# oliver-batchelor/multical

Measured on AMD Instinct MI355X. Metric: residual+Jacobian evals/sec, higher is better.
Workload: dtype f64; 1 GPU; BASELINE configs[2]: 8 cameras x 500 frames x 2 boards (charuco_16x22 + aprilgrid_9x9), rolling-shutter motion, intrinsics+extrinsics; the whole rig on 1 GPU(s); n_params=6140, n_slots=2592000, n_observations=763957, parallelism=single GPU, device=gfx950:sramecc+:xnack-:AMD Radeon Graphics:cus=256:mfma=1

## Files before the change

### multical_amd/_lib.py

```python
import ctypes as C
import os

import numpy as np

HERE = os.path.dirname(os.path.abspath(__file__))
LIB_PATH = os.environ.get("MCBA_LIB_PATH") or os.path.join(HERE, "_build", "libmcba.so")

MCBA_VERSION = 3
MOTION_STATIC, MOTION_ROLLING, MOTION_HAND_EYE = 0, 1, 2
CAMERA_PINHOLE, CAMERA_FISHEYE = 0, 1
LOSSES = dict(linear=0, soft_l1=1, huber=2, cauchy=3, arctan=4)
TR_SOLVERS = dict(exact=0, lsmr=1)
OPT_BITS = dict(camera_poses=1, board_poses=2, motion=4, cameras=8, boards=16)
PARAM_ORDER = ["camera_poses", "board_poses", "motion", "cameras", "boards"]

c_double_p = C.POINTER(C.c_double)
c_uint8_p = C.POINTER(C.c_uint8)
c_int32_p = C.POINTER(C.c_int32)


class Problem(C.Structure):
  _fields_ = [
    ("version", C.c_int32), ("n_cameras", C.c_int32), ("n_frames", C.c_int32), ("n_boards", C.c_int32),
    ("n_points", C.c_int32),
# ... 235 lines not shown
                                              c_double_p, C.POINTER(C.c_int64), c_double_p]),
  ("mcba_debug_observation_covariance_ms", C.c_int32, [H, c_double_p]),
  ("mcba_debug_set_observation_covariance_route", C.c_int32, [H, C.c_int32]),
  ("mcba_residual_gram", C.c_int32, [H, c_double_p, c_int32_p, C.c_int32, C.c_int32, C.c_int32, C.c_int32, c_double_p,
                                     C.POINTER(C.c_int64), C.POINTER(C.c_int64), C.c_int32, C.c_int32, c_int32_p]),
  ("mcba_debug_residual_gram_ms", C.c_int32, [c_double_p, C.POINTER(C.c_int64)]),
  ("mcba_warp_points", C.c_int32, [C.POINTER(FieldSet), C.c_int64, c_int32_p, C.c_int32, c_double_p, c_double_p, c_uint8_p]),
  ("mcba_undistort_maps_corrected", C.c_int32, [C.POINTER(CameraSet), C.POINTER(FieldSet), c_double_p, c_double_p, C.c_int32, C.c_int32,
                                                C.POINTER(C.c_float)]),
  ("mcba_undistort_images_corrected", C.c_int32, [C.POINTER(CameraSet), C.POINTER(FieldSet), c_double_p, c_double_p, C.c_void_p,
                                                  C.c_int32, C.c_int32, C.c_int32, C.c_int32, C.c_int32, c_int32_p, C.c_int32, C.c_int32,
                                                  C.c_double, C.c_void_p]),
  ("mcba_debug_warp_ms", C.c_int32, [c_double_p, C.POINTER(C.c_int64)]),
  ("mcba_solve", C.c_int32, [H, c_double_p, C.POINTER(Options), C.POINTER(Result)]),
  ("mcba_time_linearize", C.c_int32, [H, c_double_p, C.POINTER(Options), C.c_int32, c_double_p]),
  ("mcba_time_residuals", C.c_int32, [H, c_double_p, C.c_int32, c_double_p]),
  ("mcba_time_lsmr_iteration", C.c_int32, [H, c_double_p, C.c_int32, c_double_p]),
  ("mcba_rccl_unique_id", C.c_int32, [C.POINTER(C.c_uint8)]),
  ("mcba_rccl_init", C.c_int32, [H, C.POINTER(C.c_uint8), C.c_int32, C.c_int32]),
  ("mcba_rccl_shutdown", C.c_int32, [H]),
  ("mcba_rccl_version", C.c_int32, [C.POINTER(C.c_int32)]),
  ("mcba_set_mfma", C.c_int32, [H, C.c_int32]),
  ("mcba_debug_set_lin_grid", C.c_int32, [H, C.c_int32]),
  ("mcba_debug_set_frame_groups", C.c_int32, [H, C.c_int32]),
  ("mcba_debug_pipe_probe", C.c_int32, [C.c_int32, C.POINTER(C.c_double)]),
  ("mcba_debug_dot3", C.c_int32, [C.POINTER(C.c_double), C.POINTER(C.c_double), C.c_int64, C.POINTER(C.c_double), C.POINTER(C.c_double)]),
  ("mcba_debug_dispatch_probe", C.c_int32, [C.c_int32, C.c_int32, C.c_int32, C.c_int32, C.POINTER(C.c_longlong)]),
  ("mcba_debug_xcd_probe", C.c_int32, [C.c_int32, C.POINTER(C.c_longlong)]),
  ("mcba_debug_gn_step", C.c_int32, [H, C.c_double, c_double_p, c_double_p, c_double_p]),
  ("mcba_debug_mfma_probe", C.c_int32, [c_double_p, c_double_p]),
  ("mcba_debug_chol", C.c_int32, [H, C.c_int32, c_double_p, c_double_p, C.c_double, C.c_int32, c_double_p]),
  ("mcba_debug_linearize_profile", C.c_int32, [H, c_double_p, C.POINTER(C.c_longlong)]),
  ("mcba_debug_lsmr_products", C.c_int32, [H, c_double_p, c_double_p, c_double_p, c_double_p, c_double_p]),
  ("mcba_debug_lsmr_fused_products", C.c_int32, [H, c_double_p, c_double_p, c_double_p, c_double_p]),
  ("mcba_debug_lsmr_info", C.c_int32, [H, C.POINTER(C.c_int64)]),
  ("mcba_debug_set_lsmr_fused", C.c_int32, [H, C.c_int32]),
  ("mcba_debug_set_switch", C.c_int32, [C.c_char_p, C.c_char_p]),
  ("mcba_debug_lsmr_solve", C.c_int32, [H, c_double_p, C.POINTER(Options), C.c_double, c_double_p, C.c_int32, c_double_p, c_double_p, c_double_p]),
  ("mcba_debug_lsmr_trace", C.c_int32, [H, C.c_int32, c_double_p, C.POINTER(C.c_int32)]),
  ("mcba_debug_set_lsmr_trace", C.c_int32, [H, C.c_int32]),
  ("mcba_debug_set_lsmr_grid", C.c_int32, [H, C.c_int32]),
  ("mcba_debug_set_allreduce_trace", C.c_int32, [H, C.c_int32]),
  ("mcba_debug_set_lsmr_masks_form", C.c_int32, [H, C.c_int32]),
]

_lib = None
# ... 69 lines not shown
```

### multical_amd/backend.py

```python
import ctypes as C
import time
from types import SimpleNamespace

import numpy as np

from . import _lib
from ._lib import (Problem, Options, Result, RoundReport, LOSSES, OPT_BITS, PARAM_ORDER, MOTION_STATIC, MOTION_ROLLING,
                   MOTION_HAND_EYE, CAMERA_PINHOLE, CAMERA_FISHEYE, check, f64 as _f64)


def _ptr(a, ctype):
  return a.ctypes.data_as(C.POINTER(ctype))


def _mask_u8(a):
  a = np.asarray(a)
  if a.dtype == np.bool_ and a.flags.c_contiguous:
    return a.view(np.uint8)
  if a.dtype == np.uint8 and a.flags.c_contiguous:
    return a
  return np.ascontiguousarray(a.astype(np.uint8))


def _class_name(obj):
# ... 141 lines not shown

  def __enter__(self):
    return self

  def __exit__(self, *a):
    self.close()

  @property
  def n_residuals(self):
    n = C.c_int64()
    check(self.lib.mcba_num_residuals(self.h, C.byref(n)))
    return n.value

  def device_info(self):
    buf = C.create_string_buffer(256)
    check(self.lib.mcba_device_info(self.h, buf, 256))
    return buf.value.decode()

  def set_mfma(self, on):
    check(self.lib.mcba_set_mfma(self.h, 1 if on else 0))

  def set_lin_grid(self, grid):
    check(self.lib.mcba_debug_set_lin_grid(self.h, int(grid)))

  def set_frame_groups(self, nw):
    check(self.lib.mcba_debug_set_frame_groups(self.h, int(nw)))

  def set_inliers(self, mask):
    self._jac_pattern = None
    if mask is None:
      check(self.lib.mcba_set_inliers(self.h, None))
    else:
      m = _mask_u8(mask)
      assert m.shape == tuple(self.shape), f"inlier mask shape {m.shape} != {self.shape}"
      check(self.lib.mcba_set_inliers(self.h, _ptr(m, C.c_uint8)))

  def _x(self, x):
    x = _f64(x)
    assert x.shape == (self.n_params,), f"inconsistent parameter sizes, got {x.size}, expected {self.n_params}"
    return x

  def residuals(self, x):
    x = self._x(x)
    r = np.empty(self.n_residuals)
    check(self.lib.mcba_residuals(self.h, _ptr(x, C.c_double), _ptr(r, C.c_double)))
    return r
# ... 430 lines not shown
```

### multical_amd/csrc/mcba_api.hip

```cpp
#include <dlfcn.h>
#include <cmath>
#include <limits>

#include "../../include/mcba.h"
#include "mcba_debug.h"
#include "mcba_camops.h"
#include "mcba_dispatch.h"
#include "mcba_lower.h"
#include "mcba_solver_kernels.h"
#include "mcba_cov_kernels.h"
#include "mcba_obscov_kernels.h"
#include "mcba_residual_field_kernels.h"
#include "mcba_host.h"

using namespace mcba;
using namespace mcba::host;

namespace mcba {
namespace host {
thread_local std::string g_error;
__thread hipStream_t g_fill_stream = nullptr;
__thread bool g_park_on_release = false;
ResourceCache& resource_cache() {
  static ResourceCache* c = new ResourceCache();
  return *c;
}
}
}

static std::map<std::string, std::string>& dbg_switch_table() {
  static std::map<std::string, std::string> t;
  return t;
}
static std::mutex g_dbg_switch_mutex;
const char* mcba::host::dbg_switch(const char* name) {
  {
// ... 69 lines not shown
  DevBuf<double> comm;
  DevBuf<double> ls_u, ls_ua, ls_ub, ls_part, ls_v, ls_vraw, ls_h, ls_hbar, ls_x, ls_nrm, ls_partial, ls_out, ls_bpart, ls_comm, ls_xpart, ls_vpart, ls_part2;
  DevBuf<double2> cp_obs, cp_bxy;
  DevBuf<double> cp_bz, cp_tr;
  DevBuf<double> dot_part;
  DevBuf<int4> cp_desc;
  bool compact_dirty = true;
  DevBuf<double> ls_cache;
  int lsmr_fused_setting = -1;
  bool lsmr_masks_form = false;
  int lsmr_fused = 2;
  ScalLayout sl;
  DevBuf<double> chol_linv;
  DevBuf<double> cov_d, cov_zero, cov_x, cov_p, cov_sg, cov_sout, cov_ff, cov_fs;
  DevBuf<int32_t> cov_bad;
  DevBuf<uint8_t> oc_flag;
  DevBuf<double> oc_cov, oc_student, oc_part, oc_out, oc_g;
  double oc_pass_ms = 0.0;
  bool oc_sigma_route = false;
  DevBuf<int32_t> rf_size, rf_cov;
  DevBuf<double> rf_part, rf_gram;
  DevBuf<long long> rf_cpart, rf_count;
  int lin_grid = 0;

  int64_t n_inliers = 0;
  int64_t n_evalid = 0;

  DevBuf<double2> obs;
  DevBuf<uint8_t> inlier, evalid, fix_aspect;
  DevBuf<uint8_t> valid_fm, raw_mask, cam_valid, frame_valid, board_valid;
  DevBuf<int32_t> view_first;
  DevBuf<long long> totals;
  long long* h_totals = nullptr;
  DevBuf<int32_t> obs_index, view_count, active_views, av_counts, work_counter, board_off, full2act;
  DevBuf<double> xfull, bwg, img_h, board_points, pose, cam, view, tmat;
  DevBuf<uint16_t> tri;
  DevBuf<int4> ftab;
  int nftab = 0;
  DevBuf<long long> dbg;
  DevBuf<double> err_fm, sel_f64;
  std::vector<double> err_x;
  bool err_valid = false;
  DevBuf<unsigned int> sel_hist;
  DevBuf<unsigned long long> sel_state;
  bool obs_index_dirty = false;
  bool view_first_dirty = false;
// ... 114 lines not shown
  const Dims& d = h->d;
  h->obs_index_dirty = true; h->compact_dirty = true;
  if (d.views() > 0) {
    if (mask_ref != nullptr) {
      if (h->raw_mask.n < (size_t)d.slots()) h->raw_mask.alloc((size_t)d.slots(), false);
      upload_shard_slabs(h, h->raw_mask.p, mask_ref, 1);
      hipLaunchKernelGGL(k_lower_view, dim3(d.views()), dim3(64), 0, h->stream, d, (const double2*)nullptr, (const float2*)nullptr,
                         (const uint8_t*)h->raw_mask.p, (const uint8_t*)h->raw_mask.p, h->cam_valid.p, h->frame_valid.p,
                         h->board_valid.p, h->board_off.p, (double2*)nullptr, (uint8_t*)nullptr, (uint8_t*)nullptr,
                         h->inlier.p, h->view_count.p, (int32_t*)nullptr);
    } else {
      hipLaunchKernelGGL(k_inliers_from_valid, dim3(d.views()), dim3(64), 0, h->stream, d, h->valid_fm.p, h->inlier.p,
                         h->view_count.p);
    }
  }
  refresh_active_views(h);
  scan_views(h);
  h->out_r.alloc((size_t)std::max<int64_t>(2 * h->n_inliers, 1), false);
}

void set_loss(mcba_handle_s* h, const mcba_options* opt) {
  h->d.loss = opt ? opt->loss : MCBA_LOSS_LINEAR;
  h->d.f_scale = opt ? opt->f_scale : 1.0;
  REQUIRE(h->d.loss >= 0 && h->d.loss <= 4, "unknown loss");
  REQUIRE(h->d.loss == 0 || h->d.f_scale > 0, "f_scale must be positive");
}

void upload_x(mcba_handle_s* h, const double* x, double* dst) {
  if (h->ext2int.empty()) {
    memcpy(h->h_x, x, (size_t)h->d.n * sizeof(double));
  } else {
    memset(h->h_x, 0, (size_t)h->d.n * sizeof(double));
    for (int i = 0; i < h->n_ext; ++i) h->h_x[h->ext2int[i]] = x[i];
  }
  HIP_OK(hipMemcpyAsync(dst, h->h_x, (size_t)h->d.n * sizeof(double), hipMemcpyHostToDevice, h->stream));
}

void eval_pose_tables(mcba_handle_s* h, const double* dx) {
  const Dims& d = h->d;
  const int items = d.n_pose + d.C + d.B * d.P;
  hipLaunchKernelGGL(k_prep, dim3((items + 127) / 128), dim3(128), 0, h->stream, d, h->t, dx);
}

void eval_tables(mcba_handle_s* h, const double* dx) {
  const Dims& d = h->d;
  eval_pose_tables(h, dx);
// ... 33 lines not shown
}
void destroy_rccl_comm(void* comm) {
  if (comm && rccl_api().ok) (void)rccl_api().CommDestroy(comm);
}
int32_t rccl_allreduce_native(void* ctx, void* device_buf, size_t count, int32_t op, void* stream) {
  mcba_handle_s* h = static_cast<mcba_handle_s*>(ctx);
  const int rc = rccl_api().AllReduce(device_buf, device_buf, count,  8, op == 0 ?  0 :  2,
                                      h->rccl_comm, (hipStream_t)stream);
  return rc;
}

int call_allreduce(mcba_handle_s* h, double* buf, size_t count, int op) {
  if (!h->allreduce) return 0;
  ++h->ar_calls;
  h->ar_doubles += (int64_t)count;
  if (h->ar_trace.size() < h->ar_trace_cap) h->ar_trace.push_back(op == 0 ? (int64_t)count : -(int64_t)count);
  const int rc = h->allreduce(h->allreduce_ctx, buf, count, op, (void*)h->stream);
  if (rc != 0) throw Error("all-reduce hook failed with code " + std::to_string(rc));
  return 0;
}


void ensure_compact(mcba_handle_s* h);
LsmrCompact compact_tables(const mcba_handle_s* h);
bool linearize_table_form() {
  static const bool table = dbg_switch("MCBA_FUSED") != nullptr && atoi(dbg_switch("MCBA_FUSED")) == 0;
  return table;
}

void launch_fused_linearize_kernel(mcba_handle_s* h) {
  const Dims& d = h->d;
  static const bool masks = dbg_switch("MCBA_LIN_COMPACT") != nullptr && dbg_switch("MCBA_LIN_COMPACT")[0] == '0';
  LsmrCompact cp{nullptr, nullptr, nullptr, nullptr, nullptr};
  if (!masks) {
    ensure_compact(h);
    cp = compact_tables(h);
  }
  h->ops->linearize(d, h->t, h->stream, h->rec.p, h->tri.p, true, h->lin_grid, nullptr, h->gbuf.p, 2 * d.n + 2, h->Hss.p,
                    d.ns * d.ns, masks ? nullptr : &cp);
}

void launch_linearize(mcba_handle_s* h, const double* dx) {
  const Dims& d = h->d;
  if (!linearize_table_form() && h->use_mfma && d.off_boards < 0 && h->t.dbg == nullptr) {
    if (dx != nullptr) eval_pose_tables(h, dx);
    launch_fused_linearize_kernel(h);
    return;
  }
  const int nb_views = std::max((d.views() + TMV - 1) / TMV, 1);
  static const bool force_global = dbg_switch("MCBA_TMAT_GLOBAL") != nullptr && dbg_switch("MCBA_TMAT_GLOBAL")[0] == '1';
  const bool local = tmat_local_poses(d) <= TM_LOCAL_POSES && !force_global;
  if (dx != nullptr && !local) {
    eval_pose_tables(h, dx);
    dx = nullptr;
  }
  const int nb_prep = dx ? (d.n_pose + d.C + d.B * d.P + TM_THREADS - 1) / TM_THREADS : 0;
  if (local)
    hipLaunchKernelGGL(k_tmat<true>, dim3(nb_views + nb_prep), dim3(TM_THREADS), 0, h->stream, d, h->t, h->gbuf.p,
                       2 * d.n + 2, h->Hss.p, d.ns * d.ns, dx, nb_views);
  else
    hipLaunchKernelGGL(k_tmat<false>, dim3(nb_views), dim3(TM_THREADS), 0, h->stream, d, h->t, h->gbuf.p, 2 * d.n + 2,
                       h->Hss.p, d.ns * d.ns, (const double*)nullptr, nb_views);
  h->ops->linearize(d, h->t, h->stream, h->rec.p, h->tri.p, h->use_mfma, h->lin_grid, nullptr, nullptr, 0, nullptr, 0, nullptr);
}

constexpr size_t ASM_LDS_MAX = 150 * 1024;
inline size_t assemble_lds_fixed(const Dims& d) {
  return (size_t)frame_entries(d) * sizeof(int) + 2 * (size_t)((d.C * d.B + 3) & ~3) * sizeof(uint16_t) + 16;
}

void launch_assemble(mcba_handle_s* h, unsigned long long publish_seq = 0, int cost_slot = 0, bool step_valid = false) {
  const Dims& d = h->d;
  const int nfb = (d.DF > 0) ? d.Fl : 0;
  static const int stage_kb = dbg_switch("MCBA_ASM_STAGE_KB") ? std::min(60, std::max(4, atoi(dbg_switch("MCBA_ASM_STAGE_KB")))) : 44;
  const int ne = frame_entries(d), cb = d.C * d.B;
  const size_t fixed = assemble_lds_fixed(d);
  const size_t stage_bytes = std::min<size_t>((size_t)stage_kb * 1024, ASM_LDS_MAX - fixed);
  const int gviews = nfb ? std::max(1, std::min(cb, (int)(stage_bytes / ((size_t)ne * 8)))) : 1;
  const size_t lds = nfb ? (size_t)gviews * ne * sizeof(double) + fixed : 0;
  raise_dynamic_lds((const void*)k_assemble, h->device, lds);
  const int npair = d.C * d.B;
  static const bool force_big = dbg_switch("MCBA_SHARED_FINAL_BIG") != nullptr && dbg_switch("MCBA_SHARED_FINAL_BIG")[0] == '1';
  hipLaunchKernelGGL(k_assemble, dim3(nfb + d.C * d.B * h->nchunk), dim3(ASM_THREADS), lds, h->stream, d, h->t, h->rec.p, nfb, h->nchunk, gviews,
                     h->ftab.p, h->nftab, h->Hff.p, h->Hfs.p, h->g(), h->diag(), h->partial.p);
  check_launch("k_assemble");
  {
// ... 265 lines not shown
  const Dims& d = h->d;
  if (d.views() > 0) {
    hipLaunchKernelGGL(k_view_scan, dim3(1), dim3(1024), 0, h->stream, d, h->view_count.p, (const int32_t*)nullptr,
                       h->view_first.p, h->totals.p);
    hipLaunchKernelGGL(k_obs_index, dim3(d.views()), dim3(64), 0, h->stream, d, h->inlier.p, h->view_first.p, h->obs_index.p);
  }
  h->obs_index_dirty = false;
}

void ensure_compact(mcba_handle_s* h) {
  if (!h->compact_dirty) return;
  const Dims& d = h->d;
  ensure_view_first(h);
  const size_t n = (size_t)std::max<int64_t>(h->n_inliers, 1) + 64;
  if (h->cp_obs.n < n) { h->cp_obs.alloc(n, false); h->cp_bxy.alloc(n, false); h->cp_bz.alloc(n, false); }
  if (d.motion == MOTION_ROLLING && h->cp_tr.n < n) h->cp_tr.alloc(n, false);
  const size_t nv = std::max<size_t>(std::max(d.views(), 1), h->active_views.n > 0 ? h->active_views.n - 1 : 0);
  if (h->cp_desc.n < nv) h->cp_desc.alloc(nv, false);
  if (d.views() > 0)
    hipLaunchKernelGGL(k_compact_views, dim3((unsigned)nv), dim3(64), 0, h->stream, d, h->t, (const int32_t*)h->view_first.p, h->cp_obs.p, h->cp_bxy.p,
                       h->cp_bz.p, d.motion == MOTION_ROLLING ? h->cp_tr.p : nullptr, h->cp_desc.p);
  check_launch("k_compact_views");
  h->compact_dirty = false;
}
LsmrCompact compact_tables(const mcba_handle_s* h) {
  return LsmrCompact{h->cp_obs.p, h->cp_bxy.p, h->cp_bz.p, h->d.motion == MOTION_ROLLING ? h->cp_tr.p : nullptr, h->cp_desc.p};
}

void compute_errors(mcba_handle_s* h, const double* x) {
  const Dims& d = h->d;
  if (h->err_fm.n < (size_t)std::max(d.slots(), 1)) h->err_fm.alloc((size_t)std::max(d.slots(), 1));
  if (!h->sel_hist.p) {
    h->sel_hist.alloc((size_t)SEL_MAX * 2048);
    h->sel_state.alloc(3 * SEL_MAX + (size_t)SEL_NEXT_BLOCKS * SEL_MAX * 2);
    h->sel_f64.alloc((size_t)SEL_MAX * 2048);
  }
  const size_t nx = h->ext2int.empty() ? (size_t)d.n : (size_t)h->n_ext;
  if (h->err_valid && h->err_x.size() == nx && memcmp(h->err_x.data(), x, nx * sizeof(double)) == 0) return;
  upload_x(h, x, h->x.p);
  eval_tables(h, h->x.p);
  h->ops->residual(d, h->t, h->stream, nullptr, nullptr, nullptr, h->err_fm.p, nullptr);
  h->err_x.assign(x, x + nx);
  h->err_valid = true;
}

int sel_grid(const Dims& d) { return std::max(1, std::min(1024, (d.slots() + 255) / 256)); }
// ... 421 lines not shown
  h->shard_root = rank == 0;
  API_END
}

int32_t mcba_set_log(mcba_handle h, mcba_log_fn fn, void* ctx) {
  API_BEGIN
  REQUIRE(h, "null handle");
  h->log = fn;
  h->log_ctx = ctx;
  API_END
}

int32_t mcba_set_mfma(mcba_handle h, int32_t on) {
  API_BEGIN
  REQUIRE(h, "null handle");
  h->use_mfma = on != 0;
  API_END
}

int32_t mcba_debug_set_lin_grid(mcba_handle h, int32_t grid) {
  API_BEGIN
  REQUIRE(h && grid >= 0, "bad argument");
  h->lin_grid = grid;
  API_END
}

int32_t mcba_debug_set_frame_groups(mcba_handle h, int32_t nw) {
  API_BEGIN
  REQUIRE(h && nw >= 0 && nw <= 16, "bad argument");
  const Dims& d = h->d;
  if (nw == 0) {
    h->lin_grid = 0;
    refresh_active_views(h);
    sync(h);
    h->compact_dirty = true;
    return 0;
  }
  const int cb = d.C * d.B, nv = d.views();
  std::vector<int32_t> cnt((size_t)nv);
  HIP_OK(hipMemcpyAsync(cnt.data(), h->view_count.p, (size_t)nv * sizeof(int32_t), hipMemcpyDeviceToHost, h->stream));
  sync(h);
  std::vector<std::pair<long long, int>> frames;
  for (int fl = 0; fl < d.Fl; ++fl) {
    long long tot = 0;
    for (int k = 0; k < cb; ++k) tot += cnt[(size_t)fl * cb + k];
    if (tot > 0) frames.push_back({tot, fl});
// ... 1868 lines not shown
}

int32_t mcba_gather_inliers(mcba_handle h, uint8_t* mask) {
  API_BEGIN
  REQUIRE(h && mask, "null argument");
  g_fill_stream = h->stream;
  gather_inliers(h, mask);
  API_END
}

int32_t mcba_time_linearize(mcba_handle h, const double* x, const mcba_options* opt, int32_t repeats, double* avg_ms) {
  API_BEGIN
  REQUIRE(h && x && avg_ms && repeats > 0, "bad argument");
  set_loss(h, opt);
  upload_x(h, x, h->x.p);
  launch_linearize(h, h->x.p);
  sync(h);
  HIP_OK(hipEventRecord(h->ev0, h->stream));
  for (int i = 0; i < repeats; ++i) {
    const Dims& d = h->d;
    if (h->use_mfma && d.off_boards < 0 && !linearize_table_form())
      launch_fused_linearize_kernel(h);
    else
      h->ops->linearize(d, h->t, h->stream, h->rec.p, h->tri.p, h->use_mfma, h->lin_grid, nullptr, nullptr, 0, nullptr, 0, nullptr);
  }
  HIP_OK(hipEventRecord(h->ev1, h->stream));
  sync(h);
  float ms = 0.f;
  HIP_OK(hipEventElapsedTime(&ms, h->ev0, h->ev1));
  *avg_ms = ms / repeats;
  API_END
}

int32_t mcba_debug_lsmr_fused_products(mcba_handle h, const double* x, const double* v, double* jv_out, double* jtjv_out) {
  API_BEGIN
  REQUIRE(h && x && v && jv_out && jtjv_out, "null argument");
  REQUIRE(h->allreduce == nullptr, "single handles only");
  g_fill_stream = h->stream;
  set_loss(h, nullptr);
  const Dims& d = h->d;
  LsmrOps op = lsmr_setup(h);
  const size_t m = op.m;
  upload_x(h, x, h->x.p);
  sync(h);
  lsmr_linearize(h, h->x.p);
  std::vector<double> ones((size_t)d.n, 1.0);
  HIP_OK(hipMemcpyAsync(h->dsc.p, ones.data(), (size_t)d.n * sizeof(double), hipMemcpyHostToDevice, h->stream));
// ... 151 lines not shown
```

### multical_amd/csrc/mcba_cam_impl.h

```cpp
#include <algorithm>
#include "mcba_kernels.h"
#include "mcba_obscov_kernels.h"
#include "mcba_camops.h"
#include "mcba_dispatch.h"

namespace mcba {
namespace {

constexpr int ND_ = MCBA_ND;
constexpr int FISH_ = MCBA_FISH;

inline int slot_grid(const Dims& d) {
  const int n = d.slots();
  int g = (n + 255) / 256;
  return g < 1 ? 1 : (g > 4096 ? 4096 : g);
}

template <class F>
void with_view_shape(const Dims& d, F&& f) {
  with_motion(d.motion, [&](auto mo) { with_flag(d.KI > 0, [&](auto ok) { f(mo, ok); }); });
}

void residual(const Dims& d, const Tables& t, hipStream_t s, const int32_t* first, double* r, double* proj, double* err,
              uint8_t* valid) {
// ... 2 lines not shown
  with_flag(d.motion == MOTION_ROLLING, [&](auto roll) {
    hipLaunchKernelGGL((k_residual<ND_, FISH_, roll>), grid, block, 0, s, d, t, first, r, proj, err, valid);
  });
}

void project_model(const Dims& d, const Tables& t, hipStream_t s, int iterations, double* proj) {
  with_flag(d.motion == MOTION_ROLLING, [&](auto roll) {
    hipLaunchKernelGGL((k_project_model<ND_, FISH_, roll>), dim3(slot_grid(d)), dim3(256), 0, s, d, t, iterations, proj);
  });
}

void cost(const Dims& d, const Tables& t, hipStream_t s, double* partial, int nblk) {
  with_flag(d.motion == MOTION_ROLLING, [&](auto roll) { with_flag(d.loss != 0, [&](auto rob) {
    hipLaunchKernelGGL((k_cost<ND_, FISH_, roll, rob>), dim3(nblk), dim3(64), 0, s, d, t, partial);
  }); });
}

void jacobian(const Dims& d, const Tables& t, hipStream_t s, int row_nnz, double* vals, int32_t* cols) {
  with_flag(d.motion == MOTION_ROLLING, [&](auto roll) {
    hipLaunchKernelGGL((k_jacobian<ND_, FISH_, roll>), dim3(slot_grid(d)), dim3(128), 0, s, d, t, row_nnz, vals, cols);
  });
}

void linearize(const Dims& d, const Tables& t, hipStream_t s, double* rec, const uint16_t* tri, bool mfma, int epoch,
               const double* x, double* za, int na, double* zb, int nb, const LsmrCompact* cpp) {
  const bool fused = za != nullptr;
  const LsmrCompact cp = cpp != nullptr ? *cpp : LsmrCompact{nullptr, nullptr, nullptr, nullptr, nullptr};
  if (d.views() == 0 && !fused) return;
  const int want = epoch > 0 ? epoch : (d.views() >= 32768 ? 4 * LIN_GRID_MAX : LIN_GRID_MAX);
  const dim3 grid(std::max(1, d.views() < want ? d.views() : want)), block(64);
  const int form = !fused ? 0 : (cpp != nullptr ? 3 : 2);
  with_view_shape(d, [&](auto mo, auto ok) {
    auto launch = [&](auto mf, auto rob, auto fm, auto prof) {
      hipLaunchKernelGGL((k_linearize<ND_, FISH_, mo, ok, mf, rob, fm, prof>), grid, block, 0, s, d, t, rec, tri,
                         epoch, x, za, na, zb, nb, cp);
    };
    if (t.dbg != nullptr) launch(std::true_type{}, std::true_type{}, int_c<0>{}, std::true_type{});
    else if (!mfma) launch(std::false_type{}, std::true_type{}, int_c<0>{}, std::false_type{});
    else with_flag(d.loss != 0, [&](auto rob) { with_int<3, 2, 0>(form, [&](auto fm) {
      launch(std::true_type{}, rob, fm, std::false_type{});
    }); });
  });
}

void points(const Dims& d, const Tables& t, hipStream_t s, int nq, double* Hss, double* Hfs, double* g) {
  if (nq <= 0) return;
  with_view_shape(d, [&](auto mo, auto ok) {
    hipLaunchKernelGGL((k_points<ND_, FISH_, mo, ok>), dim3(nq), dim3(256), 0, s, d, t, Hss, Hfs, g);
  });
}

void lsmr_jv(const Dims& d, const Tables& t, hipStream_t s, const int32_t* first, int mode, const double* dscale, const double* v,
             double alpha, double* u, double* partial, int nblk, const double* ls) {
  with_view_shape(d, [&](auto mo, auto ok) { with_flag(d.loss != 0, [&](auto rob) {
    hipLaunchKernelGGL((k_lsmr_jv<ND_, FISH_, mo, ok, rob>), dim3(nblk), dim3(64), 0, s, d, t, first, mode, dscale, v, alpha, u,
                       partial, ls);
  }); });
}

void lsmr_jtu(const Dims& d, const Tables& t, hipStream_t s, const int32_t* first, double inv_beta, double* u, double* part,
              int part_stride, double* bpart, int nblk, const double* ls) {
  with_view_shape(d, [&](auto mo, auto ok) { with_flag(d.loss != 0, [&](auto rob) {
    hipLaunchKernelGGL((k_lsmr_jtu<ND_, FISH_, mo, ok, rob>), dim3(nblk), dim3(64), 0, s, d, t, first, inv_beta, u, part,
                       part_stride, bpart, ls);
  }); });
// ... 7 lines not shown
  }); });
}

void lsmr_fused2(const Dims& d, const Tables& t, hipStream_t s, const int32_t* first, const double* dscale, const double* v, double* u,
                 double* partial, double* xpart, double* part, int part_stride, double* bpart, int nblk, const double* lsIn,
                 double* lsOut, const double* vpart, int nv, double* hbar, double* x, double* h, double* cache, int mode, LsmrCompact cp) {
  with_view_shape(d, [&](auto mo, auto ok) { with_flag(d.loss != 0, [&](auto rob) { with_int<2, 3, 4, 0>(mode, [&](auto md) {
    hipLaunchKernelGGL((k_lsmr_fused2<ND_, FISH_, mo, ok, rob, md>), dim3(nblk), dim3(64), 0, s, d, t, first, dscale, v, u,
                       partial, xpart, part, part_stride, bpart, lsIn, lsOut, vpart, nv, hbar, x, h, cache, cp);
  }); }); });
}

void obs_cov(const Dims& d, const Tables& t, hipStream_t s, const double* Sss, const double* Sff, const double* Sfs, const uint8_t* pflag,
             double sigma2, double* pred_cov, double* student, double* vpart, double* out, const double* gview) {
  if (d.views() == 0) return;
  const int nblk = std::min(d.views(), 16384);
  with_view_shape(d, [&](auto mo, auto ok) {
    hipLaunchKernelGGL((k_obscov<ND_, FISH_, mo, ok>), dim3(nblk), dim3(64), 0, s, d, t, Sss, Sff, Sfs, pflag, sigma2, pred_cov,
                       student, vpart, gview);
  });
  hipLaunchKernelGGL((k_obscov_fold<1024>), dim3(1 + d.C), dim3(1024), 0, s, d, (const double*)vpart, out);
}

const CamOps OPS = {residual, project_model, cost, jacobian, linearize, points, lsmr_jv, lsmr_jtu, lsmr_fused, lsmr_fused2, obs_cov};

}

const CamOps* MCBA_CAM_FN() { return &OPS; }

}
```

### multical_amd/csrc/mcba_camops.h

```cpp
#pragma once
#include <hip/hip_runtime.h>
#include "mcba_device.h"

namespace mcba {

struct CamOps {
  void (*residual)(const Dims&, const Tables&, hipStream_t, const int32_t* first, double* r, double* proj, double* err,
                   uint8_t* valid);
  void (*project_model)(const Dims&, const Tables&, hipStream_t, int iterations, double* proj);
  void (*cost)(const Dims&, const Tables&, hipStream_t, double* partial, int nblk);
  void (*jacobian)(const Dims&, const Tables&, hipStream_t, int row_nnz, double* vals, int32_t* cols);
  void (*linearize)(const Dims&, const Tables&, hipStream_t, double* rec, const uint16_t* tri, bool mfma, int epoch,
                    const double* x, double* za, int na, double* zb, int nb, const LsmrCompact* compact);
  void (*points)(const Dims&, const Tables&, hipStream_t, int n_points, double* Hss, double* Hfs, double* g);
  void (*lsmr_jv)(const Dims&, const Tables&, hipStream_t, const int32_t* first, int mode, const double* dscale, const double* v,
                  double alpha, double* u, double* partial, int nblk, const double* ls);
  void (*lsmr_jtu)(const Dims&, const Tables&, hipStream_t, const int32_t* first, double inv_beta, double* u, double* part,
                   int part_stride, double* bpart, int nblk, const double* ls);
  void (*lsmr_fused)(const Dims&, const Tables&, hipStream_t, const int32_t* first, const double* dscale, const double* v, double* u,
                     double* partial, double* part, int part_stride, double* bpart, int nblk, const double* ls);
  void (*lsmr_fused2)(const Dims&, const Tables&, hipStream_t, const int32_t* first, const double* dscale, const double* v, double* u,
                      double* partial, double* xpart, double* part, int part_stride, double* bpart, int nblk, const double* lsIn,
                      double* lsOut, const double* vpart, int nv, double* hbar, double* x, double* h, double* cache, int mode, LsmrCompact cp);
  void (*obs_cov)(const Dims&, const Tables&, hipStream_t, const double* Sss, const double* Sff, const double* Sfs,
                  const uint8_t* pflag, double sigma2, double* pred_cov, double* student, double* vpart, double* out,
                  const double* gview );
};

const CamOps* cam_ops_pin4();
const CamOps* cam_ops_pin5();
const CamOps* cam_ops_pin8();
const CamOps* cam_ops_pin12();
const CamOps* cam_ops_pin14();
const CamOps* cam_ops_fish4();
const CamOps* cam_ops_mix14();

// ... 2 lines not shown
```

### multical_amd/csrc/mcba_debug.h

```cpp
#ifndef MCBA_DEBUG_H
#define MCBA_DEBUG_H
#include "../../include/mcba.h"
#ifdef __cplusplus
extern "C" {
#endif

int32_t mcba_set_mfma(mcba_handle h, int32_t on);
int32_t mcba_debug_set_lin_grid(mcba_handle h, int32_t grid);
int32_t mcba_debug_set_frame_groups(mcba_handle h, int32_t nw);
int32_t mcba_debug_pipe_probe(int32_t iters, double* ms_out);
int32_t mcba_debug_dot3(const double* a, const double* b, int64_t n, double* out_single, double* out_wide);
int32_t mcba_debug_dispatch_probe(int32_t blocks, int32_t threads, int32_t lds_bytes, int32_t spin, long long* out);
int32_t mcba_debug_xcd_probe(int32_t n, long long* out);
int32_t mcba_debug_gn_step(mcba_handle h, double reg, double* gn_h, double* g_h, double* scale_inv);
int32_t mcba_debug_linearize_profile(mcba_handle h, const double* x, long long* out);
int32_t mcba_debug_chol(mcba_handle h, int32_t ns, const double* S, const double* rhs, double reg, int32_t blocked,
                        double* p_out);
int32_t mcba_debug_mfma_probe(const double* V, double* out);

int32_t mcba_debug_lsmr_products(mcba_handle h, const double* x, const double* v, const double* u, double* jv_out, double* jtu_out);
int32_t mcba_debug_set_switch(const char* name, const char* value);
int32_t mcba_debug_set_lsmr_fused(mcba_handle h, int32_t on);
int32_t mcba_debug_lsmr_fused_products(mcba_handle h, const double* x, const double* v, double* jv_out, double* jtjv_out);
int32_t mcba_debug_lsmr_info(mcba_handle h, int64_t* lsmr_iterations);

int32_t mcba_debug_lsmr_solve(mcba_handle h, const double* x, const mcba_options* opt, double damp, const double* scale_in, int32_t maxiter,
                              double* gn_h_out, double* scale_out, double* out);
int32_t mcba_debug_lsmr_trace(mcba_handle h, int32_t cap, double* rows, int32_t* n_rows);
int32_t mcba_debug_set_lsmr_trace(mcba_handle h, int32_t scalars);
int32_t mcba_debug_set_lsmr_masks_form(mcba_handle h, int32_t on);
int32_t mcba_debug_set_allreduce_trace(mcba_handle h, int32_t cap);
// ... 10 lines not shown
```

### multical_amd/csrc/mcba_kernels.h

```cpp
#pragma once
#include <hip/hip_runtime.h>
#include <type_traits>
#include "mcba_view.h"
#include "mcba_lsmr.h"

namespace mcba {

typedef double double4_t __attribute__((ext_vector_type(4)));

__device__ __forceinline__ void lds_fence() {
#if defined(MCBA_EXP_LIGHT_FENCE)
  __builtin_amdgcn_wave_barrier();
#else
  __builtin_amdgcn_fence(__ATOMIC_RELEASE, "workgroup");
  __builtin_amdgcn_wave_barrier();
  __builtin_amdgcn_fence(__ATOMIC_ACQUIRE, "workgroup");
#endif
}

__device__ __forceinline__ double masked_load(const double* __restrict__ p, size_t i, bool ok) {
  return p[ok ? i : 0] * (ok ? 1.0 : 0.0);
}
__device__ __forceinline__ double masked_load_row(const double* __restrict__ row, int i, int n) {
  return row[min(i, n - 1)] * (i < n ? 1.0 : 0.0);
// ... 1173 lines not shown
    } else if (i < 24) {
      const int e = i - 18;
      const int k0 = e < 3 ? 0 : (e < 5 ? 1 : 2), k1 = e < 3 ? e : (e < 5 ? e - 2 : 2);
      Hss[(size_t)(sq + k0) * ns + sq + k1] = val;
      Hss[(size_t)(sq + k1) * ns + sq + k0] = val;
    } else if (i < 27) {
      g[gq + (i - 24)] = val;
    } else {
      const int kk = (i - 27) / 12, jj = (i - 27) % 12;
      const int gx = local_to_x(d, 0, 0, b, 6 + jj);
      if (gx >= 0) {
        const int sx = d.x_to_shared(gx);
        Hss[(size_t)(sq + kk) * ns + sx] = val;
        Hss[(size_t)sx * ns + sq + kk] = val;
      }
    }
  }
}


template <int ND, int FISH, int MOTION, bool OPTK, bool MFMA, bool ROBUST, int FUSED_MODE, bool PROF = false>
__global__ __launch_bounds__(64, (MOTION == MOTION_STATIC && !FISH && MFMA && !ROBUST && !PROF && OPTK && ND <= 5) ? 4 : 2)
void k_linearize(Dims d, Tables t, double* __restrict__ rec,
                                                     const uint16_t* __restrict__ tri, int epoch,
                                                     const double* __restrict__ x, double* __restrict__ zero_a, int na,
                                                     double* __restrict__ zero_b, int nb, LsmrCompact cp) {
  static_assert(FUSED_MODE == 0 || FUSED_MODE == 2 || FUSED_MODE == 3, "linearisation forms: 0 = table form, 2 / 3 = table-fed fused forms");
  constexpr bool FUSED = FUSED_MODE != 0;
  constexpr bool COMPACT = FUSED_MODE == 3;
  (void)x; (void)cp;
  using VS = ViewShape<ND, MOTION, OPTK>;
  constexpr bool ROLL = VS::ROLL;
  constexpr int DE = VS::DE, NPB = VS::NPB, NPC = VS::NPC, KI = VS::KI, NV = VS::NV, NT = (NV + 15) / 16, NVP = 16 * NT;
  constexpr bool NARROW = MFMA && NT == 2 && NV - 16 <= 7;
  constexpr int LDV = (NARROW ? NV : NVP) + 1;
  constexpr int SLD = NARROW ? ((NV + 1) & ~1) : NVP, SROWS = NARROW ? NV : NVP;
  constexpr int NL = NPC + KI, N1 = NL + 1;
  constexpr int ROWS = 64;
  constexpr int REC = N1 * (N1 + 1) / 2;
  constexpr int TW = NV - 16;
  constexpr bool TAILV = MFMA && NT == 2 && TW <= 7;
  constexpr int NTAIL = TAILV ? TW * (TW + 1) / 2 : 1;
  constexpr int STAGE = ROWS * LDV;
  constexpr int EPI = SLD * SROWS + (MFMA ? DE * 16 * ((NPC + 15) / 16) + (REC + 2 + 1) / 2 * 2 + 64 : 0);
  constexpr int BUF = STAGE > EPI ? STAGE : EPI;

  __shared__ __attribute__((aligned(16))) double Buf[BUF];
#if defined(MCBA_EXP_PIPE)
  constexpr bool PIPE = MFMA && !FUSED && !PROF;
#else
  constexpr bool PIPE = false;
#endif
  constexpr int NBUFS = PIPE ? 2 : 1;
  constexpr int NVS = (ROLL ? 2 : 1) * VIEW_STRIDE;
  __shared__ double TmBuf[NBUFS * DE * NPC];
  __shared__ uint16_t PidxBuf[NBUFS * LIN_MAX_POINTS];
  constexpr bool VLDS = FUSED || ROLL;
  __shared__ double VmBuf[VLDS ? NBUFS * NVS : 1];
  __shared__ double Eye3[9];
  if (threadIdx.x < 9) Eye3[threadIdx.x] = (threadIdx.x & 3) == 0 ? 1.0 : 0.0;
  double* Vbuf = Buf;
  if constexpr (FUSED) {
    for (int e = blockIdx.x * 64 + threadIdx.x; e < na; e += gridDim.x * 64) zero_a[e] = 0.0;
    for (int e = blockIdx.x * 64 + threadIdx.x; e < nb; e += gridDim.x * 64) zero_b[e] = 0.0;
  }

  const int lane = threadIdx.x;
  const int n_active = t.active_views[0];
  (void)epoch;
  constexpr int NTL = (DE * NPC + 63) / 64;
  uint8_t inb[NPB64];
  double tl[NTL], vm_f = 0.0, cam_f[5 + ND], ext_f[2];
  double camr[5 + ND], extr[CAM_STRIDE - CAM_TILT], Vr[ROLL ? 1 : NVS];
#pragma unroll
  for (int k = 0; k < CAM_STRIDE - CAM_TILT; ++k) extr[k] = 0.0;
  auto front_issue = [&](int vv, int pl) {
    const int cc = (vv / d.B) % d.C;
    if constexpr (!COMPACT) {
      const uint8_t* mrow = t.inlier + (size_t)vv * d.P;
#pragma unroll
      for (int k = 0; k < NPB64; ++k) inb[k] = masked_load_row(mrow, k * 64 + pl, d.P);
    }
    if constexpr (!FUSED) {
      const double* tg = t.tmat + (size_t)vv * (DE * NPC);
#pragma unroll
      for (int k = 0; k < NTL; ++k) tl[k] = masked_load_row(tg, k * 64 + pl, DE * NPC);
      const double* vsrc = t.view + (size_t)vv * NVS;
      if constexpr (ROLL) {
        vm_f = vsrc[min(pl, NVS - 1)];
      } else {
#pragma unroll
        for (int k = 0; k < NVS; ++k) Vr[k] = vsrc[k];
// ... 30 lines not shown
    int cnt = 0;
    if constexpr (!COMPACT) {
#pragma unroll
      for (int k = 0; k < NPB64; ++k) {
        const bool in = inb[k] != 0;
        const unsigned long long m = __ballot(in);
        if (in) pidx[cnt + __popcll(m & ((1ull << lane) - 1ull))] = (uint16_t)(k * 64 + lane);
        cnt += __popcll(m);
      }
    }
    return cnt;
  };

  int cur = 0;
  int count = 0, p_cur = 0;
  double2 ob_cur;
  ob_cur.x = ob_cur.y = 0.0;
  double X_cur[3] = {0.0, 0.0, 0.0}, X_nxt[3];
  bool front_ready = false;
  int4 dnext = make_int4(0, 0, 0, 0);
  if constexpr (COMPACT) {
    if ((int)blockIdx.x < n_active) dnext = cp.desc[blockIdx.x];
  }
  for (int vi = blockIdx.x; vi < n_active; vi += gridDim.x) {
  int v_, desc_first = 0, desc_count = 0;
  if constexpr (COMPACT) {
    v_ = dnext.x; desc_first = dnext.y; desc_count = dnext.z;
    if (vi + (int)gridDim.x < n_active) dnext = cp.desc[vi + gridDim.x];
  } else {
    v_ = t.active_views[1 + vi];
  }
  const int v = v_;
  (void)desc_first; (void)desc_count;
  if (v < 0) continue;
  const int b = v % d.B, c = (v / d.B) % d.C, fl = v / (d.B * d.C), f = d.f0 + fl;
  (void)f;
  const int vi_n = vi + (int)gridDim.x;
  const bool has_next = PIPE && vi_n < n_active;
  const int v_n = has_next ? t.active_views[1 + vi_n] : v;
  long long stamp[6] = {0, 0, 0, 0, 0, 0};
  constexpr bool prof = PROF;
  if (prof) stamp[0] = clock64();
  int pl;
  asm volatile("v_mov_b32 %0, %1" : "=v"(pl) : "v"(lane));
  double* Tm = TmBuf + cur * (DE * NPC);
  uint16_t* pidx = PidxBuf + cur * LIN_MAX_POINTS;
  double* Vm = VmBuf + (VLDS ? cur * NVS : 0);

  if (!front_ready) front_issue(v, pl);
  const double* camp = nullptr;
  if constexpr (FUSED) {
    camp = t.cam + (size_t)c * CAM_STRIDE;
    (void)camp;
    static_assert(NPB * POSE_STRIDE <= BUF, "pose entries do not fit the staging buffer");
    double* Pl = Buf;
    {
      constexpr int NPE = (NPB * POSE_STRIDE + 63) / 64;
      double pe_f[NPE];
#pragma unroll
      for (int u = 0; u < NPE; ++u) {
// ... 477 lines not shown
```

Baseline: 16380 evals/s.

## Deal compact views to linearize slots with cost-model LPT packing

Adds a host-side scheduler that estimates per-view linearization cost from observation counts, packs views onto occupancy-derived slots with LPT greedy assignment and swap refinement, and links each slot's views through the descriptor w field. The linearize kernel then launches one block per occupied slot and follows these chains instead of a grid-strided loop. The aim is to remove tail imbalance from unevenly sized views. In exchange it adds host syncs and copies whenever the schedule is rebuilt, and depends on a fixed cost model.

```diff
diff --git a/multical_amd/_lib.py b/multical_amd/_lib.py
--- a/multical_amd/_lib.py
+++ b/multical_amd/_lib.py
@@ -281,6 +281,9 @@
   ("mcba_rccl_version", C.c_int32, [C.POINTER(C.c_int32)]),
   ("mcba_set_mfma", C.c_int32, [H, C.c_int32]),
   ("mcba_debug_set_lin_grid", C.c_int32, [H, C.c_int32]),
+  ("mcba_debug_set_lin_slots", C.c_int32, [H, C.c_int32]),
+  ("mcba_debug_lin_deal_info", C.c_int32, [H, c_int32_p]),
+  ("mcba_debug_pack_slots", C.c_int32, [c_int32_p, C.c_int32, C.c_int32, C.c_int32, c_int32_p]),
   ("mcba_debug_set_frame_groups", C.c_int32, [H, C.c_int32]),
   ("mcba_debug_pipe_probe", C.c_int32, [C.c_int32, C.POINTER(C.c_double)]),
   ("mcba_debug_dot3", C.c_int32, [C.POINTER(C.c_double), C.POINTER(C.c_double), C.c_int64, C.POINTER(C.c_double), C.POINTER(C.c_double)]),
diff --git a/multical_amd/backend.py b/multical_amd/backend.py
--- a/multical_amd/backend.py
+++ b/multical_amd/backend.py
@@ -187,6 +187,20 @@
 
   def set_lin_grid(self, grid):
     check(self.lib.mcba_debug_set_lin_grid(self.h, int(grid)))
+
+  def set_lin_slots(self, slots):
+    check(self.lib.mcba_debug_set_lin_slots(self.h, int(slots)))
+
+  def lin_deal_info(self):
+    out = np.zeros(2, dtype=np.int32)
+    check(self.lib.mcba_debug_lin_deal_info(self.h, _lib.ip(out)))
+    return int(out[0]), int(out[1])
+
+  def pack_slots(self, counts, slots):
+    counts = np.ascontiguousarray(counts, dtype=np.int32)
+    out = np.empty(len(counts), dtype=np.int32)
+    check(self.lib.mcba_debug_pack_slots(_lib.ip(counts), len(counts), int(slots), 1 if self._struct.motion == MOTION_ROLLING else 0, _lib.ip(out)))
+    return out
 
   def set_frame_groups(self, nw):
     check(self.lib.mcba_debug_set_frame_groups(self.h, int(nw)))
diff --git a/multical_amd/csrc/mcba_api.hip b/multical_amd/csrc/mcba_api.hip
--- a/multical_amd/csrc/mcba_api.hip
+++ b/multical_amd/csrc/mcba_api.hip
@@ -12,6 +12,7 @@
 #include "mcba_obscov_kernels.h"
 #include "mcba_residual_field_kernels.h"
 #include "mcba_host.h"
+#include "mcba_lin_deal.h"
 
 using namespace mcba;
 using namespace mcba::host;
@@ -127,6 +128,10 @@
   DevBuf<double> rf_part, rf_gram;
   DevBuf<long long> rf_cpart, rf_count;
   int lin_grid = 0;
+  DevBuf<int4> cp_deal;
+  bool deal_dirty = true, deal_robust = false;
+  int deal_grid = 0, deal_n = 0;
+  int lin_slots = 0;
 
   int64_t n_inliers = 0;
   int64_t n_evalid = 0;
@@ -287,6 +292,7 @@
 void set_loss(mcba_handle_s* h, const mcba_options* opt) {
   h->d.loss = opt ? opt->loss : MCBA_LOSS_LINEAR;
   h->d.f_scale = opt ? opt->f_scale : 1.0;
+  if (h->deal_robust != (h->d.loss != 0)) { h->deal_robust = h->d.loss != 0; h->deal_dirty = true; }
   REQUIRE(h->d.loss >= 0 && h->d.loss <= 4, "unknown loss");
   REQUIRE(h->d.loss == 0 || h->d.f_scale > 0, "f_scale must be positive");
 }
@@ -366,6 +372,7 @@
 
 
 void ensure_compact(mcba_handle_s* h);
+void ensure_deal(mcba_handle_s* h);
 LsmrCompact compact_tables(const mcba_handle_s* h);
 bool linearize_table_form() {
   static const bool table = dbg_switch("MCBA_FUSED") != nullptr && atoi(dbg_switch("MCBA_FUSED")) == 0;
@@ -376,12 +383,17 @@
   const Dims& d = h->d;
   static const bool masks = dbg_switch("MCBA_LIN_COMPACT") != nullptr && dbg_switch("MCBA_LIN_COMPACT")[0] == '0';
   LsmrCompact cp{nullptr, nullptr, nullptr, nullptr, nullptr};
+  int deal_grid = 0, deal_n = 0;
   if (!masks) {
     ensure_compact(h);
     cp = compact_tables(h);
+    if (h->lin_grid == 0) {
+      ensure_deal(h);
+      if (h->deal_grid > 0) { cp.desc = h->cp_deal.p; deal_grid = h->deal_grid; deal_n = h->deal_n; }
+    }
   }
   h->ops->linearize(d, h->t, h->stream, h->rec.p, h->tri.p, true, h->lin_grid, nullptr, h->gbuf.p, 2 * d.n + 2, h->Hss.p,
-                    d.ns * d.ns, masks ? nullptr : &cp);
+                    d.ns * d.ns, masks ? nullptr : &cp, deal_grid, deal_n);
 }
 
 void launch_linearize(mcba_handle_s* h, const double* dx) {
@@ -405,7 +417,7 @@
   else
     hipLaunchKernelGGL(k_tmat<false>, dim3(nb_views), dim3(TM_THREADS), 0, h->stream, d, h->t, h->gbuf.p, 2 * d.n + 2,
                        h->Hss.p, d.ns * d.ns, (const double*)nullptr, nb_views);
-  h->ops->linearize(d, h->t, h->stream, h->rec.p, h->tri.p, h->use_mfma, h->lin_grid, nullptr, nullptr, 0, nullptr, 0, nullptr);
+  h->ops->linearize(d, h->t, h->stream, h->rec.p, h->tri.p, h->use_mfma, h->lin_grid, nullptr, nullptr, 0, nullptr, 0, nullptr, 0, 0);
 }
 
 constexpr size_t ASM_LDS_MAX = 150 * 1024;
@@ -717,6 +729,63 @@
                        h->cp_bz.p, d.motion == MOTION_ROLLING ? h->cp_tr.p : nullptr, h->cp_desc.p);
   check_launch("k_compact_views");
   h->compact_dirty = false;
+  h->deal_dirty = true;
+}
+
+int lin_deal_switch() {
+  static const int sw = dbg_switch("MCBA_LIN_DEAL") != nullptr ? (atoi(dbg_switch("MCBA_LIN_DEAL")) != 0 ? 1 : 0) : -1;
+  return sw;
+}
+
+void ensure_deal(mcba_handle_s* h) {
+  if (!h->deal_dirty) return;
+  const Dims& d = h->d;
+  h->deal_grid = h->deal_n = 0;
+  h->deal_dirty = false;
+  const int sw = lin_deal_switch();
+  if (sw == 0 || d.views() == 0) return;
+  if (sw < 0 && h->lin_slots == 0 && d.views() >= 32768) return;
+  const int S = h->lin_slots > 0 ? h->lin_slots : h->ops->lin_slots(d);
+  REQUIRE(S > 0, "occupancy query of k_linearize failed");
+  h->deal_dirty = true;
+  PinnedBuf count_stage(sizeof(int32_t));
+  HIP_OK(hipMemcpyAsync(count_stage.p, h->active_views.p, sizeof(int32_t), hipMemcpyDeviceToHost, h->stream));
+  sync(h);
+  const int32_t n_active = *static_cast<const int32_t*>(count_stage.p);
+  REQUIRE(n_active >= 0 && (size_t)n_active <= h->cp_desc.n, "active-view count out of range");
+  if (n_active <= S && h->lin_slots == 0) { h->deal_dirty = false; return; }
+  if (n_active == 0) { h->deal_dirty = false; return; }
+  PinnedBuf stage(2 * (size_t)n_active * sizeof(int4));
+  int4* desc = static_cast<int4*>(stage.p);
+  int4* dealt = desc + n_active;
+  HIP_OK(hipMemcpyAsync(desc, h->cp_desc.p, (size_t)n_active * sizeof(int4), hipMemcpyDeviceToHost, h->stream));
+  sync(h);
+  std::vector<int32_t> counts((size_t)n_active);
+  for (int i = 0; i < n_active; ++i) counts[i] = desc[i].x >= 0 ? desc[i].z : 0;
+  const SlotLists lists = pack_slots(counts, S, d.motion == MOTION_ROLLING ? LIN_COST_ROLLING : LIN_COST_STATIC);
+  int grid = 0;
+  for (int w = 0; w < S; ++w) grid += lists.slot_first[w + 1] > lists.slot_first[w] ? 1 : 0;
+  int head = 0, rest = grid;
+  for (int w = 0; w < S; ++w) {
+    int at = head;
+    for (int q = lists.slot_first[w]; q < lists.slot_first[w + 1]; ++q) {
+      const bool last = q + 1 == lists.slot_first[w + 1];
+      dealt[at] = desc[lists.slot_items[q]];
+      dealt[at].w = last ? 0 : rest;
+      at = rest;
+      if (!last) ++rest;
+    }
+    if (lists.slot_first[w + 1] > lists.slot_first[w]) ++head;
+  }
+  const int n = (int)lists.slot_items.size();
+  if (n > 0) {
+    if (h->cp_deal.n < (size_t)n) h->cp_deal.alloc((size_t)n, false);
+    HIP_OK(hipMemcpyAsync(h->cp_deal.p, dealt, (size_t)n * sizeof(int4), hipMemcpyHostToDevice, h->stream));
+    sync(h);
+    h->deal_grid = grid;
+    h->deal_n = n;
+  }
+  h->deal_dirty = false;
 }
 LsmrCompact compact_tables(const mcba_handle_s* h) {
   return LsmrCompact{h->cp_obs.p, h->cp_bxy.p, h->cp_bz.p, h->d.motion == MOTION_ROLLING ? h->cp_tr.p : nullptr, h->cp_desc.p};
@@ -1184,6 +1253,33 @@
   API_BEGIN
   REQUIRE(h && grid >= 0, "bad argument");
   h->lin_grid = grid;
+  API_END
+}
+
+int32_t mcba_debug_set_lin_slots(mcba_handle h, int32_t slots) {
+  API_BEGIN
+  REQUIRE(h && slots >= 0 && slots <= 65536, "bad argument");
+  h->lin_slots = slots;
+  h->deal_dirty = true;
+  API_END
+}
+
+int32_t mcba_debug_lin_deal_info(mcba_handle h, int32_t* out) {
+  API_BEGIN
+  REQUIRE(h && out, "null argument");
+  const bool on = !h->deal_dirty && !h->compact_dirty && h->lin_grid == 0;
+  out[0] = on ? h->deal_grid : 0;
+  out[1] = on ? h->deal_n : 0;
+  API_END
+}
+
+int32_t mcba_debug_pack_slots(const int32_t* counts, int32_t n, int32_t slots, int32_t rolling, int32_t* slot_of) {
+  API_BEGIN
+  REQUIRE(counts && slot_of && n >= 0 && slots > 0, "bad argument");
+  const SlotLists lists = pack_slots(std::vector<int32_t>(counts, counts + n), slots, rolling ? LIN_COST_ROLLING : LIN_COST_STATIC);
+  std::fill(slot_of, slot_of + n, -1);
+  for (int w = 0; w < slots; ++w)
+    for (int q = lists.slot_first[w]; q < lists.slot_first[w + 1]; ++q) slot_of[lists.slot_items[q]] = w;
   API_END
 }
 
@@ -3098,7 +3194,7 @@
     if (h->use_mfma && d.off_boards < 0 && !linearize_table_form())
       launch_fused_linearize_kernel(h);
     else
-      h->ops->linearize(d, h->t, h->stream, h->rec.p, h->tri.p, h->use_mfma, h->lin_grid, nullptr, nullptr, 0, nullptr, 0, nullptr);
+      h->ops->linearize(d, h->t, h->stream, h->rec.p, h->tri.p, h->use_mfma, h->lin_grid, nullptr, nullptr, 0, nullptr, 0, nullptr, 0, 0);
   }
   HIP_OK(hipEventRecord(h->ev1, h->stream));
   sync(h);
diff --git a/multical_amd/csrc/mcba_cam_impl.h b/multical_amd/csrc/mcba_cam_impl.h
--- a/multical_amd/csrc/mcba_cam_impl.h
+++ b/multical_amd/csrc/mcba_cam_impl.h
@@ -48,18 +48,19 @@
   });
 }
 
-void linearize(const Dims& d, const Tables& t, hipStream_t s, double* rec, const uint16_t* tri, bool mfma, int epoch,
-               const double* x, double* za, int na, double* zb, int nb, const LsmrCompact* cpp) {
+void linearize(const Dims& d, const Tables& t, hipStream_t s, double* rec, const uint16_t* tri, bool mfma, int grid_override,
+               const double* x, double* za, int na, double* zb, int nb, const LsmrCompact* cpp, int deal_grid, int n_dealt) {
   const bool fused = za != nullptr;
   const LsmrCompact cp = cpp != nullptr ? *cpp : LsmrCompact{nullptr, nullptr, nullptr, nullptr, nullptr};
   if (d.views() == 0 && !fused) return;
-  const int want = epoch > 0 ? epoch : (d.views() >= 32768 ? 4 * LIN_GRID_MAX : LIN_GRID_MAX);
-  const dim3 grid(std::max(1, d.views() < want ? d.views() : want)), block(64);
+  const int want = grid_override > 0 ? grid_override : (d.views() >= 32768 ? 4 * LIN_GRID_MAX : LIN_GRID_MAX);
   const int form = !fused ? 0 : (cpp != nullptr ? 3 : 2);
+  const bool dealt = form == 3 && deal_grid > 0 && n_dealt > 0;
+  const dim3 grid(dealt ? deal_grid : std::max(1, d.views() < want ? d.views() : want)), block(64);
   with_view_shape(d, [&](auto mo, auto ok) {
     auto launch = [&](auto mf, auto rob, auto fm, auto prof) {
       hipLaunchKernelGGL((k_linearize<ND_, FISH_, mo, ok, mf, rob, fm, prof>), grid, block, 0, s, d, t, rec, tri,
-                         epoch, x, za, na, zb, nb, cp);
+                         dealt ? n_dealt : 0, x, za, na, zb, nb, cp);
     };
     if (t.dbg != nullptr) launch(std::true_type{}, std::true_type{}, int_c<0>{}, std::true_type{});
     else if (!mfma) launch(std::false_type{}, std::true_type{}, int_c<0>{}, std::false_type{});
@@ -67,6 +68,17 @@
       launch(std::true_type{}, rob, fm, std::false_type{});
     }); });
   });
+}
+
+int lin_slots(const Dims& d) {
+  int per_cu = 0, dev = 0;
+  hipDeviceProp_t prop;
+  with_view_shape(d, [&](auto mo, auto ok) { with_flag(d.loss != 0, [&](auto rob) {
+    if (hipOccupancyMaxActiveBlocksPerMultiprocessor(&per_cu, k_linearize<ND_, FISH_, mo, ok, true, rob, 3, false>, 64, 0) != hipSuccess)
+      per_cu = 0;
+  }); });
+  if (per_cu <= 0 || hipGetDevice(&dev) != hipSuccess || hipGetDeviceProperties(&prop, dev) != hipSuccess) return 0;
+  return per_cu * prop.multiProcessorCount;
 }
 
 void points(const Dims& d, const Tables& t, hipStream_t s, int nq, double* Hss, double* Hfs, double* g) {
@@ -120,7 +132,7 @@
   hipLaunchKernelGGL((k_obscov_fold<1024>), dim3(1 + d.C), dim3(1024), 0, s, d, (const double*)vpart, out);
 }
 
-const CamOps OPS = {residual, project_model, cost, jacobian, linearize, points, lsmr_jv, lsmr_jtu, lsmr_fused, lsmr_fused2, obs_cov};
+const CamOps OPS = {residual, project_model, cost, jacobian, linearize, lin_slots, points, lsmr_jv, lsmr_jtu, lsmr_fused, lsmr_fused2, obs_cov};
 
 }
 
diff --git a/multical_amd/csrc/mcba_camops.h b/multical_amd/csrc/mcba_camops.h
--- a/multical_amd/csrc/mcba_camops.h
+++ b/multical_amd/csrc/mcba_camops.h
@@ -10,8 +10,9 @@
   void (*project_model)(const Dims&, const Tables&, hipStream_t, int iterations, double* proj);
   void (*cost)(const Dims&, const Tables&, hipStream_t, double* partial, int nblk);
   void (*jacobian)(const Dims&, const Tables&, hipStream_t, int row_nnz, double* vals, int32_t* cols);
-  void (*linearize)(const Dims&, const Tables&, hipStream_t, double* rec, const uint16_t* tri, bool mfma, int epoch,
-                    const double* x, double* za, int na, double* zb, int nb, const LsmrCompact* compact);
+  void (*linearize)(const Dims&, const Tables&, hipStream_t, double* rec, const uint16_t* tri, bool mfma, int grid,
+                    const double* x, double* za, int na, double* zb, int nb, const LsmrCompact* compact, int deal_grid, int n_dealt);
+  int (*lin_slots)(const Dims&);
   void (*points)(const Dims&, const Tables&, hipStream_t, int n_points, double* Hss, double* Hfs, double* g);
   void (*lsmr_jv)(const Dims&, const Tables&, hipStream_t, const int32_t* first, int mode, const double* dscale, const double* v,
                   double alpha, double* u, double* partial, int nblk, const double* ls);
diff --git a/multical_amd/csrc/mcba_debug.h b/multical_amd/csrc/mcba_debug.h
--- a/multical_amd/csrc/mcba_debug.h
+++ b/multical_amd/csrc/mcba_debug.h
@@ -7,6 +7,9 @@
 
 int32_t mcba_set_mfma(mcba_handle h, int32_t on);
 int32_t mcba_debug_set_lin_grid(mcba_handle h, int32_t grid);
+int32_t mcba_debug_set_lin_slots(mcba_handle h, int32_t slots);
+int32_t mcba_debug_lin_deal_info(mcba_handle h, int32_t* out);
+int32_t mcba_debug_pack_slots(const int32_t* counts, int32_t n, int32_t slots, int32_t rolling, int32_t* slot_of);
 int32_t mcba_debug_set_frame_groups(mcba_handle h, int32_t nw);
 int32_t mcba_debug_pipe_probe(int32_t iters, double* ms_out);
 int32_t mcba_debug_dot3(const double* a, const double* b, int64_t n, double* out_single, double* out_wide);
diff --git a/multical_amd/csrc/mcba_kernels.h b/multical_amd/csrc/mcba_kernels.h
--- a/multical_amd/csrc/mcba_kernels.h
+++ b/multical_amd/csrc/mcba_kernels.h
@@ -1219,7 +1219,7 @@
 template <int ND, int FISH, int MOTION, bool OPTK, bool MFMA, bool ROBUST, int FUSED_MODE, bool PROF = false>
 __global__ __launch_bounds__(64, (MOTION == MOTION_STATIC && !FISH && MFMA && !ROBUST && !PROF && OPTK && ND <= 5) ? 4 : 2)
 void k_linearize(Dims d, Tables t, double* __restrict__ rec,
-                                                     const uint16_t* __restrict__ tri, int epoch,
+                                                     const uint16_t* __restrict__ tri, int n_dealt,
                                                      const double* __restrict__ x, double* __restrict__ zero_a, int na,
                                                      double* __restrict__ zero_b, int nb, LsmrCompact cp) {
   static_assert(FUSED_MODE == 0 || FUSED_MODE == 2 || FUSED_MODE == 3, "linearisation forms: 0 = table form, 2 / 3 = table-fed fused forms");
@@ -1263,8 +1263,8 @@
   }
 
   const int lane = threadIdx.x;
-  const int n_active = t.active_views[0];
-  (void)epoch;
+  const bool dealt = COMPACT && n_dealt > 0;
+  const int n_active = dealt ? n_dealt : t.active_views[0];
   constexpr int NTL = (DE * NPC + 63) / 64;
   uint8_t inb[NPB64];
   double tl[NTL], vm_f = 0.0, cam_f[5 + ND], ext_f[2];
@@ -1341,11 +1341,13 @@
   if constexpr (COMPACT) {
     if ((int)blockIdx.x < n_active) dnext = cp.desc[blockIdx.x];
   }
-  for (int vi = blockIdx.x; vi < n_active; vi += gridDim.x) {
+  for (int vi = blockIdx.x, vi_n = 0; vi < n_active; vi = vi_n) {
   int v_, desc_first = 0, desc_count = 0;
+  vi_n = vi + (int)gridDim.x;
   if constexpr (COMPACT) {
     v_ = dnext.x; desc_first = dnext.y; desc_count = dnext.z;
-    if (vi + (int)gridDim.x < n_active) dnext = cp.desc[vi + gridDim.x];
+    if (dealt) vi_n = dnext.w > 0 ? dnext.w : n_active;
+    if (vi_n < n_active) dnext = cp.desc[vi_n];
   } else {
     v_ = t.active_views[1 + vi];
   }
@@ -1354,7 +1356,6 @@
   if (v < 0) continue;
   const int b = v % d.B, c = (v / d.B) % d.C, fl = v / (d.B * d.C), f = d.f0 + fl;
   (void)f;
-  const int vi_n = vi + (int)gridDim.x;
   const bool has_next = PIPE && vi_n < n_active;
   const int v_n = has_next ? t.active_views[1 + vi_n] : v;
   long long stamp[6] = {0, 0, 0, 0, 0, 0};
diff --git a/multical_amd/csrc/mcba_lin_deal.h b/multical_amd/csrc/mcba_lin_deal.h
--- /dev/null
+++ b/multical_amd/csrc/mcba_lin_deal.h
@@ -0,0 +1,99 @@
+#pragma once
+#include <stdint.h>
+#include <algorithm>
+#include <queue>
+#include <utility>
+#include <vector>
+
+namespace mcba {
+
+struct LinCostModel {
+  int fixed, chunk, tail, tail_obs;
+  long long cost(int count) const {
+    const int full = count / 64, rest = count % 64;
+    return fixed + (long long)chunk * full + (rest > 0 ? tail + (long long)tail_obs * rest : 0);
+  }
+};
+constexpr LinCostModel LIN_COST_ROLLING = {15200, 8100, 3900, 93};
+constexpr LinCostModel LIN_COST_STATIC = {6400, 6700, 4900, 50};
+
+struct SlotLists {
+  std::vector<int32_t> slot_first;
+  std::vector<int32_t> slot_items;
+  long long max_load = 0;
+};
+
+inline long long lin_list_schedule(const std::vector<std::pair<long long, int32_t>>& sorted, int S, std::vector<int32_t>* slot_of) {
+  typedef std::pair<long long, int32_t> LS;
+  std::priority_queue<LS, std::vector<LS>, std::greater<LS>> heap;
+  for (int w = 0; w < S; ++w) heap.push(LS(0, w));
+  long long mx = 0;
+  if (slot_of) slot_of->assign(sorted.size(), 0);
+  for (size_t i = 0; i < sorted.size(); ++i) {
+    LS s = heap.top();
+    heap.pop();
+    s.first += sorted[i].first;
+    mx = std::max(mx, s.first);
+    if (slot_of) (*slot_of)[i] = s.second;
+    heap.push(s);
+  }
+  return mx;
+}
+
+inline SlotLists pack_slots(const std::vector<int32_t>& counts, int S, const LinCostModel& model) {
+  SlotLists out;
+  S = std::max(S, 1);
+  std::vector<std::pair<long long, int32_t>> items;
+  for (size_t i = 0; i < counts.size(); ++i)
+    if (counts[i] > 0) items.push_back(std::make_pair(model.cost(counts[i]), (int32_t)i));
+  std::sort(items.begin(), items.end(), [](const std::pair<long long, int32_t>& a, const std::pair<long long, int32_t>& b) {
+    return a.first != b.first ? a.first > b.first : a.second < b.second;
+  });
+  std::vector<int32_t> slot_of;
+  lin_list_schedule(items, S, &slot_of);
+  std::vector<std::vector<int32_t>> lists((size_t)S);
+  std::vector<long long> load((size_t)S, 0);
+  for (size_t i = 0; i < items.size(); ++i) {
+    lists[slot_of[i]].push_back((int32_t)i);
+    load[slot_of[i]] += items[i].first;
+  }
+  for (long long round = 0, cap = 8LL * S + 64; round < cap && S > 1; ++round) {
+    int hi = 0, lo = 0;
+    for (int w = 1; w < S; ++w) {
+      if (load[w] > load[hi]) hi = w;
+      if (load[w] < load[lo]) lo = w;
+    }
+    const long long gap = load[hi] - load[lo];
+    long long best = 0;
+    int best_a = -1, best_b = -1;
+    for (size_t ia = 0; ia < lists[hi].size(); ++ia) {
+      const long long a = items[lists[hi][ia]].first;
+      for (int ib = -1; ib < (int)lists[lo].size(); ++ib) {
+        const long long t = a - (ib < 0 ? 0 : items[lists[lo][ib]].first);
+        if (t <= 0 || t >= gap) continue;
+        if (best_a < 0 || std::max(t, gap - t) < std::max(best, gap - best)) { best = t; best_a = (int)ia; best_b = ib; }
+      }
+    }
+    if (best_a < 0) break;
+    const int32_t a = lists[hi][best_a];
+    lists[hi].erase(lists[hi].begin() + best_a);
+    if (best_b >= 0) {
+      const int32_t b = lists[lo][best_b];
+      lists[lo].erase(lists[lo].begin() + best_b);
+      lists[hi].insert(std::lower_bound(lists[hi].begin(), lists[hi].end(), b), b);
+    }
+    lists[lo].insert(std::lower_bound(lists[lo].begin(), lists[lo].end(), a), a);
+    load[hi] -= best;
+    load[lo] += best;
+  }
+  out.slot_first.assign((size_t)S + 1, 0);
+  out.slot_items.reserve(items.size());
+  for (int w = 0; w < S; ++w) {
+    for (int32_t i : lists[w]) out.slot_items.push_back(items[i].second);
+    out.slot_first[w + 1] = (int32_t)out.slot_items.size();
+    out.max_load = std::max(out.max_load, load[w]);
+  }
+  return out;
+}
+
+}
```

After: 16540 evals/s, median of 6. Within noise of the previous version (+1.0%).
